# lidq92/LBDRN-MSIC

Hardware: AMD Instinct MI355X
Metric: Mpixels/s encode+decode (and bpp/PSNR parity) on D2/K5/bc64/nl2 (higher is better)
Workload: dtype f32; 1 GPU; synthetic 8-band 2048x2048 uint16 tile per step, K=5 D=2 bc=64 nl=2 bs=8192 e=10 (BASELINE.json configs[1] by default); encode fit + 16-bit weight truncation + decode; tiles_per_gpu=50, tiles_in_flight_per_gpu=4, tiles_per_launch=2, parallelism=image-sharded x1

## Files before the change

include/lbdrn_hip.h:

```cpp
#ifndef LBDRN_HIP_H
#define LBDRN_HIP_H

#include <stddef.h>
#include <stdint.h>

#ifdef __cplusplus
extern "C" {
#endif
#if defined(__GNUC__)
#pragma GCC visibility push(default)
#endif

#define LBDRN_ABI_VERSION 2

typedef enum lbdrn_status {
    LBDRN_OK = 0,
    LBDRN_E_ARG = -1,
    LBDRN_E_DEVICE = -2,
    LBDRN_E_UNSUPPORTED = -3,
    LBDRN_E_WORKSPACE = -4
} lbdrn_status;

typedef struct lbdrn_geom {
    int32_t C, H, W;
// ... 58 lines not shown

size_t lbdrn_train_workspace(const lbdrn_geom *g, const lbdrn_net *net, int32_t batch_size);
#define LBDRN_TRAIN_ALONE 0x800
int lbdrn_train_prepare(const lbdrn_geom *g, const lbdrn_net *net, const uint16_t *img,
                        const uint16_t *msb, int32_t batch_size, void *workspace,
                        size_t workspace_bytes, int32_t path, void *stream);
int lbdrn_train_epoch(const lbdrn_geom *g, const lbdrn_net *net, const uint16_t *img,
                      const uint16_t *msb, const int64_t *perm, int64_t n, int32_t batch_size,
                      float *params, float *exp_avg, float *exp_avg_sq, int64_t adam_step0,
                      double lr, float *losses, void *workspace, size_t workspace_bytes,
                      int32_t path, void *stream);

int lbdrn_train_group_max(void);
int32_t lbdrn_train_group_size(const lbdrn_geom *g, const lbdrn_net *net);
int32_t lbdrn_train_step_features(const lbdrn_geom *g, const lbdrn_net *net);
int lbdrn_train_epoch_group(int32_t count, const lbdrn_geom *const *g, const lbdrn_net *net,
                            const uint16_t *const *img, const uint16_t *const *msb, const int64_t *const *perm,
                            int64_t n, int32_t batch_size, float *const *params, float *const *exp_avg,
                            float *const *exp_avg_sq, int64_t adam_step0, double lr, float *const *losses,
                            void *const *workspace, size_t workspace_bytes, int32_t path, void *stream);

int lbdrn_train_profile_mode(int32_t mode);

size_t lbdrn_randperm_workspace(int64_t n, int32_t count);
int lbdrn_randperm(const uint64_t *seeds, int32_t count, int64_t n, int64_t *perm, void *workspace,
                   size_t workspace_bytes, void *stream);
int64_t lbdrn_mt19937_jump_poly(int32_t segment, uint32_t *poly624);

size_t lbdrn_plane_bound(int32_t C, int32_t H, int32_t W);
size_t lbdrn_plane_workspace(int32_t C, int32_t H, int32_t W);
// ... 30 lines not shown
```

lbdrn-msic_amd/csrc/cabi.hip:

```cpp
#include <string>

#include "common.hpp"

namespace lbdrn {
const char* last_error();
bool mfma_train_supported(const lbdrn_geom& g, const lbdrn_net& net, int bs = 0);
int mfma_train_step_features(const lbdrn_geom& g, const lbdrn_net& net);
bool mfma_train_takes_groups(const lbdrn_geom& g, const lbdrn_net& net);
size_t mfma_train_workspace(const lbdrn_geom& g, const lbdrn_net& net, int bs);
int mfma_train_prepare(const lbdrn_geom& g, const lbdrn_net& net, const uint16_t* img,
                       const uint16_t* msb, int bs, void* ws, size_t ws_bytes, hipStream_t s);
int mfma_train_epoch(const lbdrn_geom& g, const lbdrn_net& net, const uint16_t* img,
                     const uint16_t* msb, const int64_t* perm, int64_t n, int bs, float* params,
                     float* m, float* v, int64_t step0, double lr, float* losses, void* ws,
                     size_t ws_bytes, hipStream_t s, bool alone);
int train_profile_mode(int mode);
size_t randperm_workspace(int64_t n, int count);
size_t plane_bound(int C, int H, int W);
size_t plane_workspace(int C, int H, int W);
int plane_encode(const uint16_t* planes, int C, int H, int W, void* body, size_t body_cap, uint64_t* body_bytes,
                 void* ws, size_t ws_bytes, hipStream_t s);
int plane_decode(const void* body, size_t body_bytes, int C, int H, int W, uint16_t* planes, int* status, void* ws,
                 size_t ws_bytes, hipStream_t s);
int64_t mt19937_jump_poly(int segment, uint32_t* out);
int randperm_batch(const uint64_t* seeds, int count, int64_t n, int64_t* out, void* ws, size_t ws_bytes,
                   hipStream_t s);
int64_t jp2k_block_count(int C, int H, int W);
size_t jp2k_bound(int C, int H, int W);
size_t jp2k_workspace(int C, int H, int W);
int jp2k_encode(const uint16_t* planes, int C, int H, int W, int bits, uint8_t* out, size_t cap, size_t* nbytes, void* ws,
                size_t ws_bytes, hipStream_t s);
// ... 256 lines not shown

int lbdrn_train_group_max(void) { return 4; }

int32_t lbdrn_train_group_size(const lbdrn_geom* g, const lbdrn_net* net)
{
    if (!g || !net) return 1;
    return mfma_train_takes_groups(*g, *net) ? lbdrn_train_group_max() : 1;
}

int32_t lbdrn_train_step_features(const lbdrn_geom* g, const lbdrn_net* net)
{
    if (!g || !net) return 0;
    return mfma_train_step_features(*g, *net);
}

int lbdrn_train_epoch_group(int32_t count, const lbdrn_geom* const* g, const lbdrn_net* net, const uint16_t* const* img,
                            const uint16_t* const* msb, const int64_t* const* perm, int64_t n, int32_t batch_size,
                            float* const* params, float* const* exp_avg, float* const* exp_avg_sq, int64_t adam_step0,
                            double lr, float* const* losses, void* const* workspace, size_t workspace_bytes, int32_t path,
                            void* stream)
{
    LBDRN_REQUIRE(count >= 1 && count <= lbdrn_train_group_max(), "group of %d fits (1..%d)", count, lbdrn_train_group_max());
    LBDRN_REQUIRE(g && img && msb && perm && params && exp_avg && exp_avg_sq && workspace, "null pointer array");
    if (int rc = check_net(net)) return rc;
    for (int f = 0; f < count; ++f) {
        LBDRN_REQUIRE(g[f] && img[f] && msb[f] && perm[f] && params[f] && exp_avg[f] && exp_avg_sq[f], "null pointer (fit %d)", f);
        if (int rc = check_geom(g[f])) return rc;
        if (int rc = net_matches(g[f], net)) return rc;
        LBDRN_REQUIRE(g[f]->C == g[0]->C && g[f]->H == g[0]->H && g[f]->W == g[0]->W && g[f]->K == g[0]->K &&
                      g[f]->D == g[0]->D && g[f]->P == g[0]->P && g[f]->use_colors == g[0]->use_colors &&
// ... 116 lines not shown
```

lbdrn-msic_amd/csrc/train_mfma.hip:

```cpp
#include <atomic>
#include <cmath>
#include <cstdlib>
#include <utility>
#include <vector>

#include "common.hpp"
#include "lbdrn_math.hpp"

namespace lbdrn {

typedef float f32x4 __attribute__((ext_vector_type(4)));

constexpr int MAX_GROUP = 4;
constexpr int TB = 32;
constexpr int TBC = 64;
constexpr int HP = 68;
constexpr int TP = 36;
constexpr int OP = 20;
constexpr int RED_SLICES = 8;
constexpr int RED_LANES = 32;
constexpr int SLAB_ROT = 4;
constexpr int TRAIN_THREADS = 512;

constexpr int WB = 64;
constexpr int WAVE_THREADS = 256;
constexpr int WOP = 16;
__host__ __device__ constexpr int wave_xp(int LQ) { return LQ == 16 ? 80 : LQ == 32 ? 144 : LQ == 48 || LQ == 52 ? 208 : 272; }
constexpr int TBC_W = 64;
constexpr int WPT = 68;

struct FeatMap {
    int Fe;
    int zP, zs2, zc;
};
__host__ __device__ __forceinline__ int feat_of_slot(int j, const FeatMap& m)
{
// ... 118 lines not shown
bool mfma_train_supported(const lbdrn_geom& g, const lbdrn_net& net, int bs)
{
    TrainPlan p;
    if (make_train_plan(g, net, &p)) return bs <= 0 || slabs_addressable(p, bs);
    return wide_supported(g, net);
}

bool mfma_train_takes_groups(const lbdrn_geom& g, const lbdrn_net& net)
{
    TrainPlan p;
    return make_train_plan(g, net, &p) && p.wave == 2;
}


struct TrainWsLayout {
    size_t off_rows, off_pack, off_slab, slab_bytes, off_loss, off_stage, stage_bytes, off_map, total;
};

static TrainWsLayout train_ws_layout(const lbdrn_geom& g, const lbdrn_net& net, const TrainPlan& p, int bs)
{
    TrainWsLayout L;
    size_t o = 0;
    L.off_rows = o; o += align_up((size_t)g.H * g.W * p.RP * sizeof(float), 256);
    L.off_pack = o; o += align_up((size_t)p.pack_floats * sizeof(float), 256);
    const size_t nwg = std::max((size_t)(bs + TB - 1) / TB, 2 * ((size_t)(bs + WB - 1) / WB));
    L.slab_bytes = align_up(nwg * (size_t)p.slab_floats * sizeof(float), 256);
    L.off_slab = o; o += SLAB_ROT * L.slab_bytes;
    L.off_loss = o; o += align_up(nwg * sizeof(double), 256);
    L.stage_bytes = align_up(align_up((size_t)bs, WB) * p.RP * sizeof(float), 256);
    L.off_stage = o; o += 2 * L.stage_bytes;
    L.off_map = o; o += align_up((size_t)p.slab_floats * 4 * sizeof(int), 256);
    L.total = o;
    return L;
}

static bool slabs_addressable(const TrainPlan& p, int bs)
{
    const size_t nwg = std::max((size_t)(bs + TB - 1) / TB, 2 * ((size_t)(bs + WB - 1) / WB));
    return nwg * (size_t)p.slab_floats * sizeof(float) < ((size_t)1 << 31);
}

size_t mfma_train_workspace(const lbdrn_geom& g, const lbdrn_net& net, int bs)
// ... 222 lines not shown

constexpr int RED_AUX = 0x00;
#ifdef LBDRN_TIMELINE
constexpr int TL_SLOTS = 2048;
__device__ __forceinline__ void timeline_store(unsigned long long* tl, int slot, bool drain)
{
    if (!tl || slot >= TL_SLOTS) return;
    unsigned long long t;
    if (drain) asm volatile("s_waitcnt vmcnt(0)" ::: "memory");
    asm volatile("s_memrealtime %0\n\ts_waitcnt lgkmcnt(0)" : "=s"(t)::"memory");
    tl[slot] = t;
}
#endif
struct ReduceFit {
    const float* slabs;
    float *params, *m, *v, *packed;
    const double* loss_part;
    float* loss_out;
};
struct ReduceArgs {
    ReduceFit fit[MAX_GROUP];
    unsigned long long* tl;
    int nloss;
};

__global__ void __launch_bounds__(RED_SLICES * RED_LANES)
    k_reduce_adam(ReduceArgs R, int nwg, int slab_floats, const int4* __restrict__ map, float step_size, float bc2_sqrt,
                  double loss_count, int pairs)
{
    __shared__ __attribute__((aligned(16))) float part[RED_SLICES][4 * RED_LANES];
    __builtin_amdgcn_s_setprio(3);
#ifdef LBDRN_TIMELINE
    if (threadIdx.x == 0 && blockIdx.x == 0 && blockIdx.y == 0) timeline_store(R.tl, 1, false);
#endif
    const ReduceFit& F = R.fit[blockIdx.y];
    const float* __restrict__ slabs = F.slabs;
    float* __restrict__ params = F.params;
    float* __restrict__ m = F.m;
    float* __restrict__ v = F.v;
    float* __restrict__ packed = F.packed;
    const int l16 = threadIdx.x % RED_LANES, slice = threadIdx.x / RED_LANES;
    const int base = blockIdx.x * (4 * RED_LANES);
    int4 me = make_int4(-1, -1, -1, 0);
    float pm = 0.f, pv = 0.f, pp = 0.f;
    if (threadIdx.x < 4 * RED_LANES) {
        me = map[base + threadIdx.x];
        const int j = me.x < 0 ? 0 : me.x;
        pm = m[j]; pv = v[j]; pp = params[j];
    }
    const int per = (nwg + RED_SLICES - 1) / RED_SLICES;
    const int w0 = slice * per, w1 = min(nwg, w0 + per);
    float4 acc = make_float4(0.f, 0.f, 0.f, 0.f);
    const __amdgpu_buffer_rsrc_t srs = __builtin_amdgcn_make_buffer_rsrc(const_cast<float*>(slabs), (short)0,
                                                                         (int)((size_t)nwg * (pairs ? 2 : 1) * slab_floats * 4), 0x00020000);
    const int voff = (base + 4 * l16) * 4;
    auto slab4 = [&](int slab) -> float4 {
        typedef int v4i __attribute__((ext_vector_type(4)));
        const v4i x = __builtin_amdgcn_raw_buffer_load_b128(srs, voff + slab * slab_floats * 4, 0, RED_AUX);
        return make_float4(__int_as_float(x[0]), __int_as_float(x[1]), __int_as_float(x[2]), __int_as_float(x[3]));
    };
    int w = w0;
    if (pairs) {
        for (; w + 8 <= w1; w += 8) {
            float4 t[8], o[8];
#pragma unroll
            for (int u = 0; u < 8; ++u) {
                t[u] = slab4(2 * (w + u));
                o[u] = slab4(2 * (w + u) + 1);
            }
#pragma unroll
            for (int u = 0; u < 8; ++u) { acc.x += t[u].x + o[u].x; acc.y += t[u].y + o[u].y; acc.z += t[u].z + o[u].z; acc.w += t[u].w + o[u].w; }
        }
        for (; w < w1; ++w) {
            const float4 t = slab4(2 * w), o = slab4(2 * w + 1);
            acc.x += t.x + o.x; acc.y += t.y + o.y; acc.z += t.z + o.z; acc.w += t.w + o.w;
        }
    }
    for (; w + 16 <= w1; w += 16) {
        float4 t[16];
#pragma unroll
        for (int u = 0; u < 16; ++u) t[u] = slab4(w + u);
#pragma unroll
        for (int u = 0; u < 16; ++u) { acc.x += t[u].x; acc.y += t[u].y; acc.z += t[u].z; acc.w += t[u].w; }
    }
    for (; w < w1; ++w) {
        const float4 t = slab4(w);
        acc.x += t.x; acc.y += t.y; acc.z += t.z; acc.w += t.w;
    }
    *reinterpret_cast<float4*>(&part[slice][4 * l16]) = acc;
    __syncthreads();
    if (threadIdx.x < 4 * RED_LANES && me.x >= 0) {
        float g = part[0][threadIdx.x];
#pragma unroll
        for (int s = 1; s < RED_SLICES; ++s) g += part[s][threadIdx.x];
        const float w1c = (float)(1.0 - 0.9), b2 = 0.999f, w2c = (float)(1.0 - 0.999), eps = 1e-8f;
        float mi = pm + w1c * (g - pm);
        float vi = pv * b2 + w2c * (g * g);
        float denom = __builtin_sqrtf(vi) / bc2_sqrt + eps;
        float pi = pp + (-step_size) * (mi / denom);
        m[me.x] = mi;
        v[me.x] = vi;
        params[me.x] = pi;
        if (me.y >= 0) packed[me.y] = pi;
        if (me.z >= 0) packed[me.z] = pi;
    }
    if (blockIdx.x == 0 && threadIdx.x == 0 && F.loss_out) {
        double s = 0.0;
        if (pairs) for (int k = 0; k + 1 < R.nloss; k += 2) s += F.loss_part[k] + F.loss_part[k + 1];
        else for (int k = 0; k < R.nloss; ++k) s += F.loss_part[k];
        *F.loss_out = (float)(s / loss_count);
    }
#ifdef LBDRN_TIMELINE
    __syncthreads();
    if (threadIdx.x == 0 && blockIdx.y == 0) timeline_store(R.tl, 514 + blockIdx.x, true);
#endif
}

static void launch_reduce(const ReduceArgs& R, int blocks, int count, bool pairs, int nwg, int slab_floats, const int4* map,
                          float step_size, float bc2_sqrt, double loss_count, hipStream_t s)
{
    k_reduce_adam<<<dim3((unsigned)blocks, (unsigned)count), RED_SLICES * RED_LANES, 0, s>>>(R, nwg, slab_floats, map, step_size, bc2_sqrt,
                                                                                            loss_count, pairs ? 1 : 0);
}


struct TrainFit {
    const float* rows;
    const int64_t* perm;
    const float* params;
    const float* packed;
    float* slabs;
    double* loss_part;
};
struct TrainArgs {
    lbdrn_net net;
    TrainPlan p;
    int64_t npix;
// ... 27 lines not shown
typedef int v4i32 __attribute__((ext_vector_type(4)));
struct WtBuf {
    __amdgpu_buffer_rsrc_t r;
    float* base;
    __device__ __forceinline__ WtBuf(float* p, size_t bytes) : base(p)
    {
        r = __builtin_amdgcn_make_buffer_rsrc(p, (short)0, (int)bytes, 0x00020000);
    }
    __device__ __forceinline__ void store_plain(int float_off, float a, float b, float c, float d) const
    {
        *reinterpret_cast<float4*>(base + float_off) = make_float4(a, b, c, d);
    }
    __device__ __forceinline__ void store(int float_off, float a, float b, float c, float d) const
    {
        v4i32 v = {__float_as_int(a), __float_as_int(b), __float_as_int(c), __float_as_int(d)};
        __builtin_amdgcn_raw_buffer_store_b128(v, r, float_off * 4, 0, 16 );
    }
};

template <int N>
__device__ __forceinline__ void lds_load(const float* src, float (&dst)[N])
{
#pragma unroll
    for (int g = 0; g < N / 4; ++g) {
        float4 v = *reinterpret_cast<const float4*>(src + 4 * g);
        dst[4 * g] = v.x; dst[4 * g + 1] = v.y; dst[4 * g + 2] = v.z; dst[4 * g + 3] = v.w;
    }
}

template <int LQ, int NL>
__global__ void __launch_bounds__(TRAIN_THREADS, 2) k_train_mfma(TrainArgs A)
// ... 555 lines not shown
        return LBDRN_E_WORKSPACE;
    }
    A.net = net; A.npix = (int64_t)g.H * g.W;
    ReduceArgs R;
    for (int f = 0; f < MAX_GROUP; ++f) {
        const int k = f < count ? f : 0;
        if (!ws[k]) { set_error("null train workspace"); return LBDRN_E_WORKSPACE; }
        float* packed = (float*)((char*)ws[k] + L.off_pack);
        A.fit[f].rows = (float*)((char*)ws[k] + L.off_rows);
        A.fit[f].params = params[k];
        A.fit[f].packed = packed;
        A.fit[f].slabs = (float*)((char*)ws[k] + L.off_slab);
        A.fit[f].loss_part = (double*)((char*)ws[k] + L.off_loss);
        A.fit[f].perm = perm[k];
        R.fit[f].slabs = A.fit[f].slabs; R.fit[f].params = params[k]; R.fit[f].m = m[k]; R.fit[f].v = v[k];
        R.fit[f].packed = packed; R.fit[f].loss_part = A.fit[f].loss_part; R.fit[f].loss_out = nullptr;
        if (f < count) {
            LBDRN_HIP_TRY(hipMemsetAsync(packed, 0, (size_t)A.p.pack_floats * sizeof(float), s));
            k_pack_train<<<(unsigned)((A.p.NP + 255) / 256), 256, 0, s>>>(params[k], A.p, net.F, net.nl, net.C, packed);
            LBDRN_LAUNCH_CHECK();
        }
    }
    int4* map = (int4*)((char*)ws[0] + L.off_map);
    k_build_map<<<(unsigned)((A.p.slab_floats + 255) / 256), 256, 0, s>>>(A.p, net.F, net.nl, net.C, map);
    LBDRN_LAUNCH_CHECK();
    float* stage[2] = {(float*)((char*)ws[0] + L.off_stage), (float*)((char*)ws[0] + L.off_stage + L.stage_bytes)};
    A.stamps = nullptr;
#ifdef LBDRN_TRAIN_STAMPS
    const int max_wg = (bs + TB - 1) / TB;
    LBDRN_HIP_TRY(hipMalloc(&A.stamps, (size_t)max_wg * 8 * 16 * sizeof(unsigned long long)));
#endif
    A.tl = nullptr; R.tl = nullptr;
#ifdef LBDRN_TIMELINE
    const int tl_steps = (int)((n + bs - 1) / bs);
    unsigned long long* tl_buf = nullptr;
    {
        LBDRN_HIP_TRY(hipMalloc(&tl_buf, (size_t)tl_steps * TL_SLOTS * sizeof(unsigned long long)));
        LBDRN_HIP_TRY(hipMemset(tl_buf, 0, (size_t)tl_steps * TL_SLOTS * sizeof(unsigned long long)));
    }
#endif
    const int rows_per_wg = A.p.wave ? WB : TB;
    const bool split = (alone && count == 1 && split_available(A.p, net)) || split_only(A.p);
    const int red_blocks = A.p.slab_floats / (4 * RED_LANES);
    int64_t step = step0;
    int si = 0;
    for (int64_t first = 0; first < n; first += bs, ++si) {
        const int B = (int)std::min<int64_t>(bs, n - first);
        const int nwg = (B + rows_per_wg - 1) / rows_per_wg;
        for (int f = 0; f < MAX_GROUP; ++f) {
            const int k = f < count ? f : 0;
            A.fit[f].perm = perm[k] + first;
            R.fit[f].loss_out = (f < count && losses && losses[k]) ? losses[k] + si : nullptr;
        }
        A.batch_n = B;
        for (int f = 0; f < MAX_GROUP; ++f) {
            const int k = f < count ? f : 0;
            A.fit[f].slabs = (float*)((char*)ws[k] + L.off_slab + (size_t)(si % SLAB_ROT) * L.slab_bytes);
            R.fit[f].slabs = A.fit[f].slabs;
        }
#ifdef LBDRN_TIMELINE
        A.tl = tl_buf + (size_t)TL_SLOTS * si; R.tl = A.tl;
#endif
        A.inv = 1.0f / ((float)B * (float)net.C);
        const int64_t nextB = std::max<int64_t>(0, std::min<int64_t>(bs, n - first - bs));
        A.stage_in = si > 0 ? stage[si & 1] : nullptr;
        A.stage_out = nextB > 0 ? stage[(si + 1) & 1] : nullptr;
        if (A.p.wave) A.stage_in = nullptr, A.stage_out = nullptr;
        A.perm_next = perm[0] + first + bs;
        A.next_n = (int)nextB;
        A.touch_row_bytes = (alone && count == 1) ? TOUCH_ROW_BYTES : 0;
        const bool split_now = split && (B >= 2 || split_only(A.p));
        auto train_launch = [&]() { return split_now ? dispatch_split(A, 2 * nwg, count, s) : dispatch_train(A, nwg, count, s); };
        if (int rc = train_launch()) return rc;
        if (g_prof_mode == 2)
            if (int rc = train_launch()) return rc;
        ++step;
        const double bc1 = 1.0 - std::pow(0.9, (double)step), bc2 = 1.0 - std::pow(0.999, (double)step);
        R.nloss = split_now ? 2 * nwg : nwg;
        if (g_prof_mode != 3 && g_prof_mode != 4)
                launch_reduce(R, red_blocks, count, split_now, nwg, A.p.slab_floats, map, (float)(lr / bc1), (float)std::sqrt(bc2), (double)B * net.C, s);
        if (g_prof_mode == 1) {
            ReduceArgs R0 = R;
            for (int f = 0; f < MAX_GROUP; ++f) R0.fit[f].loss_out = nullptr;
            launch_reduce(R0, red_blocks, count, split_now, nwg, A.p.slab_floats, map, 0.0f, (float)std::sqrt(bc2), (double)B * net.C, s);
        }
        LBDRN_LAUNCH_CHECK();
    }
#ifdef LBDRN_TIMELINE
    {
        LBDRN_HIP_TRY(hipStreamSynchronize(s));
        std::vector<unsigned long long> h((size_t)tl_steps * TL_SLOTS);
        LBDRN_HIP_TRY(hipMemcpy(h.data(), tl_buf, h.size() * sizeof(unsigned long long), hipMemcpyDeviceToHost));
        (void)hipFree(tl_buf);
        double tr = 0, g1 = 0, rd = 0, g2 = 0; int cnt = 0;
        auto last = [&](int k, int lo, int hi) { unsigned long long m = 0; for (int j = lo; j < hi; ++j) m = std::max(m, h[(size_t)k * TL_SLOTS + j]); return m; };
        for (int k = 8; k + 1 < tl_steps; ++k) {
            const unsigned long long ts = h[(size_t)k * TL_SLOTS], rs = h[(size_t)k * TL_SLOTS + 1], te = last(k, 2, 514), re = last(k, 514, TL_SLOTS);
            const unsigned long long ts2 = h[(size_t)(k + 1) * TL_SLOTS];
            tr += (double)(te - ts); g1 += (double)((long long)(rs - te)); rd += (double)(re - rs); g2 += (double)((long long)(ts2 - re));
// ... 75 lines not shown
```

lbdrn-msic_amd/csrc/train_split.inc:

```
constexpr int SPB = 32;
constexpr int SP_HP = 68;
constexpr int SP_OP = 20;
constexpr int SP_PT = 36;
constexpr int SP_SM = 40;

constexpr int SP_RING = 12;
__host__ __device__ constexpr bool split_ring(int LQ) { return LQ > 64; }
__host__ __device__ constexpr int split_w0_groups(int LQ) { return split_ring(LQ) ? SP_RING : LQ / 4; }
__host__ __device__ constexpr int split_small_through(int k, int SPI) { return k * SPI < SP_SM / 4 ? k * SPI : SP_SM / 4; }

struct SplitLds { int w0, sm, x, xt, h0, red, idx, bias, h1, e, zo, zt, total; };
__host__ __device__ constexpr SplitLds split_lds(int LQ)
{
    SplitLds L{};
    const int G0 = LQ / 4, RG = split_w0_groups(LQ);
    int o = 0;
    const int over = 2 * SPB * SP_HP + SPB * SP_OP + 2 * 64 * SP_PT;
    L.w0 = o; o += RG * 4 * 256 > over ? RG * 4 * 256 : over;
    L.sm = o; o += SP_SM * 256;
    L.xt = (G0 + 1) * SGP + 16;
    L.x = o; o += 2 * L.xt;
    L.h0 = o; o += SPB * SP_HP;
    L.red = o; o += 4 + 4 * 16 + 12;
    L.idx = o; o += 4 * 256;
// ... 43 lines not shown
    const int tid = threadIdx.x, lane = tid & 63;
    const int wv = __builtin_amdgcn_readfirstlane(tid >> 6);
    const int st = wv >> 1, uh = wv & 1;
    const int i = lane & 15, q = lane >> 4;
    const int C = A.net.C;
    const float* W0s = lds + L.w0;
    const float* SMs = lds + L.sm;
    const float* Xs = lds + L.x;
    float* H0 = lds + L.h0;
    float* H1 = lds + L.h1;
    float* E = lds + L.e;
    float* Zo = lds + L.zo;
    float* ZT = lds + L.zt;
    float* red = lds + L.red;
    const unsigned lds0 = (unsigned)(size_t)(__attribute__((address_space(3))) void*)lds;
    const int wg = blockIdx.x, grp = wg >> 1, par = wg & 1;
    const int qb = (i >> 2) & 1, jr = (i & 3) + 4 * (i >> 3);
    const int rho = 16 * (2 * st + qb) + 2 * jr + par;
    const int grow = grp * WB + rho;
    const bool live = grow < A.batch_n;
    const int srow = 16 * st + i;
    const int sig = 8 * (2 * st + qb) + jr;
    const int t0 = 2 * uh;
    float* slab = F.slabs + (size_t)wg * p.slab_floats;
    const WtBuf slabw(slab, (size_t)p.slab_floats * 4);
#ifdef LBDRN_TRAIN_STAMPS
    unsigned long long stamp[16] = {};
    asm volatile("s_memrealtime %0\n\ts_waitcnt lgkmcnt(0)" : "=s"(stamp[14])::"memory");
#endif
#ifdef LBDRN_TIMELINE
    if (lane == 0 && wv == 0 && wg == 0 && blockIdx.y == 0) timeline_store(A.tl, 0, false);
// ... 363 lines not shown
            slab[p.sl_bias + TBC_W + 16 * w + lane] = s1;
        }
    }
    if (w == 3 && lane < 16)
        slab[p.sl_bias + NL * TBC_W + lane] = (red[4 + lane] + red[20 + lane]) + (red[36 + lane] + red[52 + lane]);
    asm volatile("" ::"v"(touched));
    STAMP(11); STAMP(12);
#ifdef LBDRN_TIMELINE
    if (lane == 0 && uh == 0 && blockIdx.y == 0) timeline_store(A.tl, 2 + 2 * wg + st, true);
#endif
#ifdef LBDRN_TRAIN_STAMPS
    asm volatile("s_waitcnt vmcnt(0)" ::: "memory");
    STAMP(13);
    asm volatile("s_memrealtime %0\n\ts_waitcnt lgkmcnt(0)" : "=s"(stamp[15])::"memory");
    if (lane == 0 && A.stamps)
        for (int k = 0; k < 16; ++k) A.stamps[(((size_t)blockIdx.y * gridDim.x + wg) * 4 + wv) * 16 + k] = stamp[k];
#endif
}
```

lbdrn-msic_amd/csrc/train_stream.inc:

```
constexpr int SGP = 260;
__host__ __device__ constexpr int stream_groups(int LQ) { return LQ / 4 + 1; }
__host__ __device__ constexpr int stream_rp(int LQ) { return 16 * stream_groups(LQ); }
__host__ __device__ constexpr int stream_wpx(int LQ)
{
    const int n = stream_groups(LQ) * SGP;
    return n + ((16 - n % 32) + 32) % 32;
}
constexpr int SHP = 68, SOP = 20;
constexpr int SHSZ = WB * SHP + 48;
constexpr int SZOSZ = WB * SOP + 48;
constexpr int SZTSZ = TBC_W * WPT;

constexpr int SRED = 8 + 2 * 64;
struct StreamLds { int x, stage, h0, red, h1, zo, zt, wh, wht, idx, total, small; };
__host__ __device__ constexpr StreamLds stream_lds(int LQ, int NL)
{
    StreamLds L{};
    const int G0 = LQ / 4, NST = (G0 + 2) / 2;
    L.x = 0;
    L.stage = 4 * stream_wpx(LQ);
    const int stage_end = L.stage + 4 * G0 * 256;
    const bool alias = 2 * (NST - 1) - 1 >= (SHSZ + SRED + 1023) / 1024 - 1;
    int r = alias ? L.stage + ((SHSZ + SRED + 3) & ~3) : L.stage;
    L.h1 = r; r += (NL - 1) * SHSZ;
// ... 149 lines not shown
    constexpr bool SMALL = L.small != 0;
    constexpr int NH = (NL - 1) * 16;
    static_assert(L.total * 4 <= 160 * 1024, "LDS map does not fit");
    const int tid = threadIdx.x, lane = tid & 63;
    const int w = __builtin_amdgcn_readfirstlane(tid >> 6);
    const int i = lane & 15, q = lane >> 4;
    const int C = A.net.C;
    float* Xs = lds + L.x;
    const float* ST = lds + L.stage;
    float* H0 = lds + L.h0;
    float* red = lds + L.red;
    float* ZT = lds + L.zt;
    float* Zo = lds + L.zo;
    auto Hl = [&](int l) -> float* { return l == 0 ? H0 : lds + L.h1 + (size_t)(l - 1) * SHSZ; };
    const unsigned lds0 = (unsigned)(size_t)(__attribute__((address_space(3))) void*)lds;
    const int wg = blockIdx.x, first = wg * WB;
    const int nvalid = min(WB, A.batch_n - first);
    const int srow = 16 * w + i;
    float* slab = F.slabs + (size_t)wg * p.slab_floats;
    const WtBuf slabw(slab, (size_t)p.slab_floats * 4);
    if (w == 4) {
        const float* fsrc = F.packed + p.pk_w0 + lane * 4;
        auto issue_frags = [&](int s) {
#pragma unroll
            for (int g = 2 * s; g < 2 * s + 2; ++g)
                if (g < G0)
#pragma unroll
                    for (int t = 0; t < 4; ++t) stream_dma(fsrc + 256 * (t * G0 + g), lds0 + 4u * (unsigned)(L.stage + (g * 4 + t) * 256));
        };
        if (A.batch_n >= 2) {
            const int64_t* isrc = F.perm + min(first + 2 * (lane & 31), A.batch_n - 2);
// ... 576 lines not shown
            if (half == 0) slab[p.sl_bias + u] = mine + other;
        }
        if (w == 3 && lane < 16)
            slab[p.sl_bias + NL * TBC_W + lane] = ((red[8 + lane] + red[24 + lane]) + (red[40 + lane] + red[56 + lane])) +
                                                  ((red[72 + lane] + red[88 + lane]) + (red[104 + lane] + red[120 + lane]));
    }
    STAMP(12);
#ifdef LBDRN_TIMELINE
    if (lane == 0 && blockIdx.y == 0) timeline_store(A.tl, 2 + wg * 4 + w, true);
#endif
#ifdef LBDRN_TRAIN_STAMPS
    asm volatile("s_waitcnt vmcnt(0)" ::: "memory");
    STAMP(13);
    asm volatile("s_memrealtime %0\n\ts_waitcnt lgkmcnt(0)" : "=s"(stamp[15])::"memory");
    if (lane == 0 && A.stamps)
        for (int k = 0; k < 16; ++k) A.stamps[(((size_t)blockIdx.y * gridDim.x + wg) * 4 + w) * 16 + k] = stamp[k];
#endif
}
```

lbdrn-msic_amd/csrc/train_wide.inc:

```

struct WidePlan {
    FeatMap fm;
    int LQ, NT0, RP, NT, bc, nl;
    int64_t NP;
    int64_t offW[3], offB[3];
    int pk_w0, pk_wh, pk_wl, pk_wht, pk_wlt, pack_floats;
    int sl_hid, sl_out, sl_bias, slab_floats;
    int w_dp, w_df;
    int lds_floats;
    int xo;
};

constexpr int DW_KS = 1024;
constexpr int HB = 32;

static bool make_wide_plan(const lbdrn_geom& g, const lbdrn_net& net, WidePlan* out)
{
    if (net.act != LBDRN_ACT_SINE || (net.bc != 128 && net.bc != 256) || net.nl < 1 || net.nl > 2 || net.C > 16 || net.F < 1) return false;
    WidePlan p;
    p.bc = net.bc; p.NT = net.bc / 16; p.nl = net.nl;
    p.fm = centre_skipping_map(g, net);
    p.RP = (p.fm.Fe + net.C + 3) / 4 * 4;
    p.LQ = 0;
    for (int lq : {16, 32, 48, 52, 64})
// ... 27 lines not shown
    p.w_dp = 64 / rp4;
    p.w_df = 64 % rp4;
    p.xo = (16 * p.NT0 + 63) / 64 * 64;
    {
        const int ep = net.bc + 4, r0 = std::max(HB * wave_xp(p.LQ), HB * ep);
        p.lds_floats = r0 + (net.nl > 1 ? HB * ep : 0) + 2 * HB * 20 + 4;
    }
    if ((size_t)p.lds_floats * 4 > 160 * 1024) return false;
    if (p.xo > 256) return false;
    *out = p;
    return true;
}

static int wide_plan_features(const WidePlan& p) { return p.fm.Fe; }

struct WideWsLayout { size_t off_rows, off_pack, off_slab, off_loss, off_map, off_x, off_h[2], off_dz[2], off_dzo, total; };

static WideWsLayout wide_ws_layout(const lbdrn_geom& g, const lbdrn_net& net, const WidePlan& p, int bs)
{
    WideWsLayout L;
    size_t o = 0;
    const size_t rpw = HB;
    const size_t nwg = ((size_t)bs + rpw - 1) / rpw;
    L.off_rows = o; o += align_up((size_t)g.H * g.W * p.RP * sizeof(float), 256);
    L.off_pack = o; o += align_up((size_t)p.pack_floats * sizeof(float), 256);
    const size_t nrows = (nwg * rpw + 63) / 64 * 64, nslabs = (nrows + DW_KS - 1) / DW_KS;
    L.off_slab = o; o += align_up(nslabs * (size_t)p.slab_floats * sizeof(float), 256);
    L.off_loss = o; o += align_up(nwg * sizeof(double), 256);
    L.off_map = o; o += align_up((size_t)p.slab_floats * 4 * sizeof(int), 256);
    L.off_x = o; o += align_up(nrows * (size_t)p.xo * sizeof(float), 256);
    L.off_h[1] = L.off_dz[1] = o;
    for (int l = 0; l < net.nl; ++l) {
        L.off_h[l] = o; o += align_up(nrows * (size_t)p.bc * sizeof(float), 256);
        L.off_dz[l] = o; o += align_up(nrows * (size_t)p.bc * sizeof(float), 256);
    }
    L.off_dzo = o; o += align_up(nrows * (size_t)WOP * sizeof(float), 256);
    L.total = o;
    return L;
}

__device__ __forceinline__ int2 wide_frag_pos(int64_t idx, const WidePlan& p, int F, int C)
{
// ... 727 lines not shown
        A.batch_n = B;
        A.inv = 1.0f / ((float)B * (float)net.C);
        if (int rc = dispatch_wide(A, nwg, s, false)) return rc;
        if (g_prof_mode == 2)
            if (int rc = dispatch_wide(A, nwg, s, false)) return rc;
        Dw.nrows = (nwg * rpw + 63) / 64 * 64;
        const int nslabs = Dw.nslices = (Dw.nrows + DW_KS - 1) / DW_KS;
        if (g_prof_mode != 4)
            if (int rc = dispatch_dw(Dw, s)) return rc;
        if (g_prof_mode == 5)
            if (int rc = dispatch_dw(Dw, s)) return rc;
        ++step;
        const double bc1 = 1.0 - std::pow(0.9, (double)step), bc2 = 1.0 - std::pow(0.999, (double)step);
        ReduceArgs R;
        for (int f = 0; f < MAX_GROUP; ++f)
            R.fit[f] = ReduceFit{A.slabs, params, m, v, packed, A.loss_part, losses ? losses + si : nullptr};
        R.nloss = nwg;
        R.tl = nullptr;
        if (g_prof_mode != 3 && g_prof_mode != 4)
            launch_reduce(R, A.p.slab_floats / (4 * RED_LANES), 1, false, nslabs, A.p.slab_floats, map, (float)(lr / bc1), (float)std::sqrt(bc2), (double)B * net.C, s);
        if (g_prof_mode == 1) {
            for (int f = 0; f < MAX_GROUP; ++f) R.fit[f].loss_out = nullptr;
            launch_reduce(R, A.p.slab_floats / (4 * RED_LANES), 1, false, nslabs, A.p.slab_floats, map, 0.0f, (float)std::sqrt(bc2), (double)B * net.C, s);
        }
        LBDRN_LAUNCH_CHECK();
    }
#ifdef LBDRN_TRAIN_STAMPS
    {
        LBDRN_HIP_TRY(hipStreamSynchronize(s));
        const int nw = ((int)std::min<int64_t>(bs, n) + HB - 1) / HB * 4;
        std::vector<unsigned long long> h((size_t)nw * 16);
        LBDRN_HIP_TRY(hipMemcpy(h.data(), A.stamps, h.size() * sizeof(unsigned long long), hipMemcpyDeviceToHost));
        (void)hipFree(A.stamps);
        double d[14] = {}, clk = 0;
        for (int k = 0; k < nw; ++k) {
            for (int j = 1; j <= 13; ++j) d[j] += (double)(h[k * 16 + j] - h[k * 16 + j - 1]);
            clk += (double)(h[k * 16 + 13] - h[k * 16 + 0]) / (double)(h[k * 16 + 15] - h[k * 16 + 14]) * 100.0;
        }
// ... 11 lines not shown
```

lbdrn-msic_amd/lbdrn_hip/_lib.py:

```python
import ctypes
import os

_HERE = os.path.dirname(os.path.abspath(__file__))
_LIB_PATH = os.environ.get("LBDRN_HIP_LIB") or os.path.join(os.path.dirname(_HERE), "liblbdrn_hip.so")

ABI_VERSION = 2
PATH_AUTO, PATH_GENERIC, PATH_MFMA = 0, 1, 2
EVAL_BACKGROUND = 0x200
EVAL_FAST = 0x400
EVAL_X16 = 0x1000
TRAIN_ALONE = 0x800


class LbdrnError(RuntimeError):
    code = None


E_ARG, E_DEVICE, E_UNSUPPORTED, E_WORKSPACE = -1, -2, -3, -4


class Geom(ctypes.Structure):
    _fields_ = [("C", ctypes.c_int32), ("H", ctypes.c_int32), ("W", ctypes.c_int32),
                ("K", ctypes.c_int32), ("D", ctypes.c_int32), ("msb_max", ctypes.c_int32),
                ("use_colors", ctypes.c_int32), ("relative", ctypes.c_int32),
# ... 22 lines not shown
    "lbdrn_forward": (ctypes.c_int, [_NP, _vp, _vp, _i64, _vp, _vp, _sz, _vp]),
    "lbdrn_tape_bytes": (_sz, [_NP, _i64]),
    "lbdrn_forward_tape": (ctypes.c_int, [_NP, _vp, _vp, _i64, _vp, _vp, _sz, _vp]),
    "lbdrn_backward_workspace": (_sz, [_NP, _i64]),
    "lbdrn_backward": (ctypes.c_int, [_NP, _vp, _vp, _i64, _vp, _sz, _vp, _vp, _vp, _vp, _vp, _sz, _vp]),
    "lbdrn_apply_workspace": (_sz, [_GP, _NP]),
    "lbdrn_decode_fused": (ctypes.c_int, [_GP, _NP, _vp, _vp, _vp, _vp, _vp, _sz, _i32, _vp]),
    "lbdrn_eval_sse": (ctypes.c_int, [_GP, _NP, _vp, _vp, _vp, _vp, _vp, _sz, _i32, _vp]),
    "lbdrn_train_workspace": (_sz, [_GP, _NP, _i32]),
    "lbdrn_train_prepare": (ctypes.c_int, [_GP, _NP, _vp, _vp, _i32, _vp, _sz, _i32, _vp]),
    "lbdrn_train_epoch": (ctypes.c_int, [_GP, _NP, _vp, _vp, _vp, _i64, _i32, _vp, _vp, _vp, _i64,
                                         _dbl, _vp, _vp, _sz, _i32, _vp]),
    "lbdrn_train_group_max": (ctypes.c_int, []),
    "lbdrn_train_step_features": (_i32, [_GP, _NP]),
    "lbdrn_train_group_size": (_i32, [_GP, _NP]),
    "lbdrn_train_epoch_group": (ctypes.c_int, [_i32, _vp, _NP, _vp, _vp, _vp, _i64, _i32, _vp, _vp, _vp, _i64, _dbl, _vp,
                                               _vp, _sz, _i32, _vp]),
    "lbdrn_train_profile_mode": (ctypes.c_int, [_i32]),
    "lbdrn_randperm_workspace": (_sz, [_i64, _i32]),
    "lbdrn_randperm": (ctypes.c_int, [ctypes.POINTER(ctypes.c_uint64), _i32, _i64, _vp, _vp, _sz, _vp]),
    "lbdrn_mt19937_jump_poly": (_i64, [_i32, _vp]),
    "lbdrn_plane_bound": (_sz, [_i32, _i32, _i32]),
    "lbdrn_plane_workspace": (_sz, [_i32, _i32, _i32]),
    "lbdrn_plane_encode": (ctypes.c_int, [_vp, _i32, _i32, _i32, _vp, _sz, _vp, _vp, _sz, _vp]),
    "lbdrn_plane_decode": (ctypes.c_int, [_vp, _sz, _i32, _i32, _i32, _vp, _vp, _vp, _sz, _vp]),
    "lbdrn_jp2k_block_count": (_i64, [_i32, _i32, _i32]),
    "lbdrn_jp2k_bound": (_sz, [_i32, _i32, _i32]),
    "lbdrn_jp2k_workspace": (_sz, [_i32, _i32, _i32]),
    "lbdrn_jp2k_encode": (ctypes.c_int, [_vp, _i32, _i32, _i32, _i32, _vp, _sz, ctypes.POINTER(ctypes.c_size_t), _vp, _sz, _vp]),
    "lbdrn_weights_bound": (_sz, [_i64]),
# ... 41 lines not shown
```

Before: 69.30 Mpixels/s.

## Split gradient slab reduction into parallel slice kernel plus Adam kernel, reorder workgroups

Replaces the single reduce+Adam kernel, which had each block loop over all slabs for 8 slices, with a first kernel that spreads slice partial sums across many small blocks and writes them to a new partial buffer. A second kernel sums the 8 partials and applies Adam, and when there are only a few slabs it reads them directly and skips the first kernel. Training workgroups are renumbered so consecutive block IDs map to different reduction slices, with an early exit for padding blocks. This aims to increase parallelism in the reduction, at the cost of an extra launch and extra global traffic for the partial buffer.

```diff
diff --git a/include/lbdrn_hip.h b/include/lbdrn_hip.h
--- a/include/lbdrn_hip.h
+++ b/include/lbdrn_hip.h
@@ -96,6 +96,8 @@
 int lbdrn_train_group_max(void);
 int32_t lbdrn_train_group_size(const lbdrn_geom *g, const lbdrn_net *net);
 int32_t lbdrn_train_step_features(const lbdrn_geom *g, const lbdrn_net *net);
+int32_t lbdrn_train_slice_grid(int32_t groups, int32_t split);
+int32_t lbdrn_train_slice_workgroup(int32_t groups, int32_t split, int32_t index);
 int lbdrn_train_epoch_group(int32_t count, const lbdrn_geom *const *g, const lbdrn_net *net,
                             const uint16_t *const *img, const uint16_t *const *msb, const int64_t *const *perm,
                             int64_t n, int32_t batch_size, float *const *params, float *const *exp_avg,
diff --git a/lbdrn-msic_amd/csrc/cabi.hip b/lbdrn-msic_amd/csrc/cabi.hip
--- a/lbdrn-msic_amd/csrc/cabi.hip
+++ b/lbdrn-msic_amd/csrc/cabi.hip
@@ -15,6 +15,8 @@
                      float* m, float* v, int64_t step0, double lr, float* losses, void* ws,
                      size_t ws_bytes, hipStream_t s, bool alone);
 int train_profile_mode(int mode);
+int train_slice_grid(int groups, bool split);
+int train_slice_workgroup(int groups, bool split, int b);
 size_t randperm_workspace(int64_t n, int count);
 size_t plane_bound(int C, int H, int W);
 size_t plane_workspace(int C, int H, int W);
@@ -301,6 +303,9 @@
     return mfma_train_step_features(*g, *net);
 }
 
+int32_t lbdrn_train_slice_grid(int32_t groups, int32_t split) { return train_slice_grid(groups, split != 0); }
+int32_t lbdrn_train_slice_workgroup(int32_t groups, int32_t split, int32_t index) { return train_slice_workgroup(groups, split != 0, index); }
+
 int lbdrn_train_epoch_group(int32_t count, const lbdrn_geom* const* g, const lbdrn_net* net, const uint16_t* const* img,
                             const uint16_t* const* msb, const int64_t* const* perm, int64_t n, int32_t batch_size,
                             float* const* params, float* const* exp_avg, float* const* exp_avg_sq, int64_t adam_step0,
diff --git a/lbdrn-msic_amd/csrc/train_mfma.hip b/lbdrn-msic_amd/csrc/train_mfma.hip
--- a/lbdrn-msic_amd/csrc/train_mfma.hip
+++ b/lbdrn-msic_amd/csrc/train_mfma.hip
@@ -19,7 +19,28 @@
 constexpr int OP = 20;
 constexpr int RED_SLICES = 8;
 constexpr int RED_LANES = 32;
-constexpr int SLAB_ROT = 4;
+constexpr int RED_COLS = 64;
+#ifndef AB_SLAB_ROT
+#define AB_SLAB_ROT 4
+#endif
+#ifndef AB_STORE_AUX
+#define AB_STORE_AUX 16
+#endif
+constexpr int SLAB_ROT = AB_SLAB_ROT;
+__host__ __device__ __forceinline__ int slice_per(int groups) { return (groups + RED_SLICES - 1) / RED_SLICES; }
+__host__ __device__ __forceinline__ int slice_group(int b, int per) { return (b % RED_SLICES) * per + b / RED_SLICES; }
+__host__ __device__ __forceinline__ int slice_split_wg(int b, int per)
+{
+    const int j = b / RED_SLICES;
+    return 2 * ((b % RED_SLICES) * per + (j >> 1)) + (j & 1);
+}
+int train_slice_grid(int groups, bool split) { return groups < 1 ? 0 : RED_SLICES * slice_per(groups) * (split ? 2 : 1); }
+int train_slice_workgroup(int groups, bool split, int b)
+{
+    if (groups < 1 || b < 0 || b >= train_slice_grid(groups, split)) return -1;
+    const int per = slice_per(groups), wg = split ? slice_split_wg(b, per) : slice_group(b, per);
+    return (split ? wg >> 1 : wg) < groups ? wg : -1;
+}
 constexpr int TRAIN_THREADS = 512;
 
 constexpr int WB = 64;
@@ -168,7 +189,7 @@
 
 
 struct TrainWsLayout {
-    size_t off_rows, off_pack, off_slab, slab_bytes, off_loss, off_stage, stage_bytes, off_map, total;
+    size_t off_rows, off_pack, off_slab, slab_bytes, off_part, off_loss, off_stage, stage_bytes, off_map, total;
 };
 
 static TrainWsLayout train_ws_layout(const lbdrn_geom& g, const lbdrn_net& net, const TrainPlan& p, int bs)
@@ -180,6 +201,7 @@
     const size_t nwg = std::max((size_t)(bs + TB - 1) / TB, 2 * ((size_t)(bs + WB - 1) / WB));
     L.slab_bytes = align_up(nwg * (size_t)p.slab_floats * sizeof(float), 256);
     L.off_slab = o; o += SLAB_ROT * L.slab_bytes;
+    L.off_part = o; o += align_up((size_t)RED_SLICES * p.slab_floats * sizeof(float), 256);
     L.off_loss = o; o += align_up(nwg * sizeof(double), 256);
     L.stage_bytes = align_up(align_up((size_t)bs, WB) * p.RP * sizeof(float), 256);
     L.off_stage = o; o += 2 * L.stage_bytes;
@@ -432,6 +454,7 @@
 #endif
 struct ReduceFit {
     const float* slabs;
+    float* part;
     float *params, *m, *v, *packed;
     const double* loss_part;
     float* loss_out;
@@ -442,39 +465,25 @@
     int nloss;
 };
 
-__global__ void __launch_bounds__(RED_SLICES * RED_LANES)
-    k_reduce_adam(ReduceArgs R, int nwg, int slab_floats, const int4* __restrict__ map, float step_size, float bc2_sqrt,
-                  double loss_count, int pairs)
-{
-    __shared__ __attribute__((aligned(16))) float part[RED_SLICES][4 * RED_LANES];
+__global__ void __launch_bounds__(RED_COLS)
+    k_reduce_slices(ReduceArgs R, int nwg, int slab_floats, int pairs)
+{
     __builtin_amdgcn_s_setprio(3);
 #ifdef LBDRN_TIMELINE
     if (threadIdx.x == 0 && blockIdx.x == 0 && blockIdx.y == 0) timeline_store(R.tl, 1, false);
 #endif
     const ReduceFit& F = R.fit[blockIdx.y];
-    const float* __restrict__ slabs = F.slabs;
-    float* __restrict__ params = F.params;
-    float* __restrict__ m = F.m;
-    float* __restrict__ v = F.v;
-    float* __restrict__ packed = F.packed;
-    const int l16 = threadIdx.x % RED_LANES, slice = threadIdx.x / RED_LANES;
-    const int base = blockIdx.x * (4 * RED_LANES);
-    int4 me = make_int4(-1, -1, -1, 0);
-    float pm = 0.f, pv = 0.f, pp = 0.f;
-    if (threadIdx.x < 4 * RED_LANES) {
-        me = map[base + threadIdx.x];
-        const int j = me.x < 0 ? 0 : me.x;
-        pm = m[j]; pv = v[j]; pp = params[j];
-    }
-    const int per = (nwg + RED_SLICES - 1) / RED_SLICES;
+    const int slice = blockIdx.x % RED_SLICES, lane4 = (blockIdx.x / RED_SLICES) * RED_COLS + threadIdx.x;
+    if (4 * lane4 >= slab_floats) return;
+    const int per = slice_per(nwg);
     const int w0 = slice * per, w1 = min(nwg, w0 + per);
     float4 acc = make_float4(0.f, 0.f, 0.f, 0.f);
-    const __amdgpu_buffer_rsrc_t srs = __builtin_amdgcn_make_buffer_rsrc(const_cast<float*>(slabs), (short)0,
+    const __amdgpu_buffer_rsrc_t srs = __builtin_amdgcn_make_buffer_rsrc(const_cast<float*>(F.slabs), (short)0,
                                                                          (int)((size_t)nwg * (pairs ? 2 : 1) * slab_floats * 4), 0x00020000);
-    const int voff = (base + 4 * l16) * 4;
+    const int voff = 16 * lane4;
     auto slab4 = [&](int slab) -> float4 {
         typedef int v4i __attribute__((ext_vector_type(4)));
-        const v4i x = __builtin_amdgcn_raw_buffer_load_b128(srs, voff + slab * slab_floats * 4, 0, RED_AUX);
+        const v4i x = __builtin_amdgcn_raw_buffer_load_b128(srs, voff, slab * slab_floats * 4, RED_AUX);
         return make_float4(__int_as_float(x[0]), __int_as_float(x[1]), __int_as_float(x[2]), __int_as_float(x[3]));
     };
     int w = w0;
@@ -505,12 +514,31 @@
         const float4 t = slab4(w);
         acc.x += t.x; acc.y += t.y; acc.z += t.z; acc.w += t.w;
     }
-    *reinterpret_cast<float4*>(&part[slice][4 * l16]) = acc;
-    __syncthreads();
-    if (threadIdx.x < 4 * RED_LANES && me.x >= 0) {
-        float g = part[0][threadIdx.x];
-#pragma unroll
-        for (int s = 1; s < RED_SLICES; ++s) g += part[s][threadIdx.x];
+    *reinterpret_cast<float4*>(F.part + (size_t)slice * slab_floats + 4 * lane4) = acc;
+}
+
+__global__ void __launch_bounds__(4 * RED_LANES)
+    k_reduce_adam(ReduceArgs R, int nparts, int slab_floats, const int4* __restrict__ map, float step_size, float bc2_sqrt,
+                  double loss_count, int pairs)
+{
+
+    __builtin_amdgcn_s_setprio(3);
+    const ReduceFit& F = R.fit[blockIdx.y];
+    float* __restrict__ params = F.params;
+    float* __restrict__ m = F.m;
+    float* __restrict__ v = F.v;
+    float* __restrict__ packed = F.packed;
+    const int e = blockIdx.x * (4 * RED_LANES) + threadIdx.x;
+    const int4 me = map[e];
+    if (me.x >= 0) {
+        const float pm = m[me.x], pv = v[me.x], pp = params[me.x];
+        float p8[RED_SLICES];
+#pragma unroll
+        for (int s = 0; s < RED_SLICES; ++s)
+            p8[s] = nparts == 0 ? F.part[(size_t)s * slab_floats + e] : s < nparts ? 0.0f + F.slabs[(size_t)s * slab_floats + e] : 0.0f;
+        float g = p8[0];
+#pragma unroll
+        for (int s = 1; s < RED_SLICES; ++s) g += p8[s];
         const float w1c = (float)(1.0 - 0.9), b2 = 0.999f, w2c = (float)(1.0 - 0.999), eps = 1e-8f;
         float mi = pm + w1c * (g - pm);
         float vi = pv * b2 + w2c * (g * g);
@@ -529,16 +557,18 @@
         *F.loss_out = (float)(s / loss_count);
     }
 #ifdef LBDRN_TIMELINE
-    __syncthreads();
     if (threadIdx.x == 0 && blockIdx.y == 0) timeline_store(R.tl, 514 + blockIdx.x, true);
 #endif
 }
 
-static void launch_reduce(const ReduceArgs& R, int blocks, int count, bool pairs, int nwg, int slab_floats, const int4* map,
+static void launch_reduce(const ReduceArgs& R, int count, bool pairs, int nwg, int slab_floats, const int4* map,
                           float step_size, float bc2_sqrt, double loss_count, hipStream_t s)
 {
-    k_reduce_adam<<<dim3((unsigned)blocks, (unsigned)count), RED_SLICES * RED_LANES, 0, s>>>(R, nwg, slab_floats, map, step_size, bc2_sqrt,
-                                                                                            loss_count, pairs ? 1 : 0);
+    const int cols = (slab_floats / 4 + RED_COLS - 1) / RED_COLS;
+    const bool direct = !pairs && nwg <= RED_SLICES;
+    if (!direct) k_reduce_slices<<<dim3((unsigned)(RED_SLICES * cols), (unsigned)count), RED_COLS, 0, s>>>(R, nwg, slab_floats, pairs ? 1 : 0);
+    k_reduce_adam<<<dim3((unsigned)(slab_floats / (4 * RED_LANES)), (unsigned)count), 4 * RED_LANES, 0, s>>>(R, direct ? nwg : 0, slab_floats, map, step_size,
+                                                                                                         bc2_sqrt, loss_count, pairs ? 1 : 0);
 }
 
 
@@ -596,7 +626,7 @@
     __device__ __forceinline__ void store(int float_off, float a, float b, float c, float d) const
     {
         v4i32 v = {__float_as_int(a), __float_as_int(b), __float_as_int(c), __float_as_int(d)};
-        __builtin_amdgcn_raw_buffer_store_b128(v, r, float_off * 4, 0, 16 );
+        __builtin_amdgcn_raw_buffer_store_b128(v, r, float_off * 4, 0, AB_STORE_AUX);
     }
 };
 
@@ -1182,7 +1212,7 @@
         A.fit[f].loss_part = (double*)((char*)ws[k] + L.off_loss);
         A.fit[f].perm = perm[k];
         R.fit[f].slabs = A.fit[f].slabs; R.fit[f].params = params[k]; R.fit[f].m = m[k]; R.fit[f].v = v[k];
-        R.fit[f].packed = packed; R.fit[f].loss_part = A.fit[f].loss_part; R.fit[f].loss_out = nullptr;
+        R.fit[f].packed = packed; R.fit[f].part = (float*)((char*)ws[k] + L.off_part); R.fit[f].loss_part = A.fit[f].loss_part; R.fit[f].loss_out = nullptr;
         if (f < count) {
             LBDRN_HIP_TRY(hipMemsetAsync(packed, 0, (size_t)A.p.pack_floats * sizeof(float), s));
             k_pack_train<<<(unsigned)((A.p.NP + 255) / 256), 256, 0, s>>>(params[k], A.p, net.F, net.nl, net.C, packed);
@@ -1209,7 +1239,6 @@
 #endif
     const int rows_per_wg = A.p.wave ? WB : TB;
     const bool split = (alone && count == 1 && split_available(A.p, net)) || split_only(A.p);
-    const int red_blocks = A.p.slab_floats / (4 * RED_LANES);
     int64_t step = step0;
     int si = 0;
     for (int64_t first = 0; first < n; first += bs, ++si) {
@@ -1238,7 +1267,9 @@
         A.next_n = (int)nextB;
         A.touch_row_bytes = (alone && count == 1) ? TOUCH_ROW_BYTES : 0;
         const bool split_now = split && (B >= 2 || split_only(A.p));
-        auto train_launch = [&]() { return split_now ? dispatch_split(A, 2 * nwg, count, s) : dispatch_train(A, nwg, count, s); };
+        auto train_launch = [&]() {
+            return split_now ? dispatch_split(A, train_slice_grid(nwg, true), count, s) : dispatch_train(A, A.p.wave == 2 ? train_slice_grid(nwg, false) : nwg, count, s);
+        };
         if (int rc = train_launch()) return rc;
         if (g_prof_mode == 2)
             if (int rc = train_launch()) return rc;
@@ -1246,11 +1277,11 @@
         const double bc1 = 1.0 - std::pow(0.9, (double)step), bc2 = 1.0 - std::pow(0.999, (double)step);
         R.nloss = split_now ? 2 * nwg : nwg;
         if (g_prof_mode != 3 && g_prof_mode != 4)
-                launch_reduce(R, red_blocks, count, split_now, nwg, A.p.slab_floats, map, (float)(lr / bc1), (float)std::sqrt(bc2), (double)B * net.C, s);
+                launch_reduce(R, count, split_now, nwg, A.p.slab_floats, map, (float)(lr / bc1), (float)std::sqrt(bc2), (double)B * net.C, s);
         if (g_prof_mode == 1) {
             ReduceArgs R0 = R;
             for (int f = 0; f < MAX_GROUP; ++f) R0.fit[f].loss_out = nullptr;
-            launch_reduce(R0, red_blocks, count, split_now, nwg, A.p.slab_floats, map, 0.0f, (float)std::sqrt(bc2), (double)B * net.C, s);
+            launch_reduce(R0, count, split_now, nwg, A.p.slab_floats, map, 0.0f, (float)std::sqrt(bc2), (double)B * net.C, s);
         }
         LBDRN_LAUNCH_CHECK();
     }
diff --git a/lbdrn-msic_amd/csrc/train_split.inc b/lbdrn-msic_amd/csrc/train_split.inc
--- a/lbdrn-msic_amd/csrc/train_split.inc
+++ b/lbdrn-msic_amd/csrc/train_split.inc
@@ -81,7 +81,9 @@
     float* ZT = lds + L.zt;
     float* red = lds + L.red;
     const unsigned lds0 = (unsigned)(size_t)(__attribute__((address_space(3))) void*)lds;
-    const int wg = blockIdx.x, grp = wg >> 1, par = wg & 1;
+    const int ngrp = (A.batch_n + WB - 1) / WB;
+    const int wg = slice_split_wg(blockIdx.x, slice_per(ngrp)), grp = wg >> 1, par = wg & 1;
+    if (grp >= ngrp) return;
     const int qb = (i >> 2) & 1, jr = (i & 3) + 4 * (i >> 3);
     const int rho = 16 * (2 * st + qb) + 2 * jr + par;
     const int grow = grp * WB + rho;
@@ -475,6 +477,6 @@
     STAMP(13);
     asm volatile("s_memrealtime %0\n\ts_waitcnt lgkmcnt(0)" : "=s"(stamp[15])::"memory");
     if (lane == 0 && A.stamps)
-        for (int k = 0; k < 16; ++k) A.stamps[(((size_t)blockIdx.y * gridDim.x + wg) * 4 + wv) * 16 + k] = stamp[k];
+        for (int k = 0; k < 16; ++k) A.stamps[(((size_t)blockIdx.y * 2 * ngrp + wg) * 4 + wv) * 16 + k] = stamp[k];
 #endif
 }
diff --git a/lbdrn-msic_amd/csrc/train_stream.inc b/lbdrn-msic_amd/csrc/train_stream.inc
--- a/lbdrn-msic_amd/csrc/train_stream.inc
+++ b/lbdrn-msic_amd/csrc/train_stream.inc
@@ -187,7 +187,9 @@
     float* Zo = lds + L.zo;
     auto Hl = [&](int l) -> float* { return l == 0 ? H0 : lds + L.h1 + (size_t)(l - 1) * SHSZ; };
     const unsigned lds0 = (unsigned)(size_t)(__attribute__((address_space(3))) void*)lds;
-    const int wg = blockIdx.x, first = wg * WB;
+    const int ngrp = (A.batch_n + WB - 1) / WB;
+    const int wg = slice_group(blockIdx.x, slice_per(ngrp)), first = wg * WB;
+    if (wg >= ngrp) return;
     const int nvalid = min(WB, A.batch_n - first);
     const int srow = 16 * w + i;
     float* slab = F.slabs + (size_t)wg * p.slab_floats;
@@ -794,6 +796,6 @@
     STAMP(13);
     asm volatile("s_memrealtime %0\n\ts_waitcnt lgkmcnt(0)" : "=s"(stamp[15])::"memory");
     if (lane == 0 && A.stamps)
-        for (int k = 0; k < 16; ++k) A.stamps[(((size_t)blockIdx.y * gridDim.x + wg) * 4 + w) * 16 + k] = stamp[k];
+        for (int k = 0; k < 16; ++k) A.stamps[(((size_t)blockIdx.y * ngrp + wg) * 4 + w) * 16 + k] = stamp[k];
 #endif
 }
diff --git a/lbdrn-msic_amd/csrc/train_wide.inc b/lbdrn-msic_amd/csrc/train_wide.inc
--- a/lbdrn-msic_amd/csrc/train_wide.inc
+++ b/lbdrn-msic_amd/csrc/train_wide.inc
@@ -65,7 +65,7 @@
 
 static int wide_plan_features(const WidePlan& p) { return p.fm.Fe; }
 
-struct WideWsLayout { size_t off_rows, off_pack, off_slab, off_loss, off_map, off_x, off_h[2], off_dz[2], off_dzo, total; };
+struct WideWsLayout { size_t off_rows, off_pack, off_slab, off_part, off_loss, off_map, off_x, off_h[2], off_dz[2], off_dzo, total; };
 
 static WideWsLayout wide_ws_layout(const lbdrn_geom& g, const lbdrn_net& net, const WidePlan& p, int bs)
 {
@@ -77,6 +77,7 @@
     L.off_pack = o; o += align_up((size_t)p.pack_floats * sizeof(float), 256);
     const size_t nrows = (nwg * rpw + 63) / 64 * 64, nslabs = (nrows + DW_KS - 1) / DW_KS;
     L.off_slab = o; o += align_up(nslabs * (size_t)p.slab_floats * sizeof(float), 256);
+    L.off_part = o; o += align_up((size_t)RED_SLICES * p.slab_floats * sizeof(float), 256);
     L.off_loss = o; o += align_up(nwg * sizeof(double), 256);
     L.off_map = o; o += align_up((size_t)p.slab_floats * 4 * sizeof(int), 256);
     L.off_x = o; o += align_up(nrows * (size_t)p.xo * sizeof(float), 256);
@@ -834,14 +835,14 @@
         const double bc1 = 1.0 - std::pow(0.9, (double)step), bc2 = 1.0 - std::pow(0.999, (double)step);
         ReduceArgs R;
         for (int f = 0; f < MAX_GROUP; ++f)
-            R.fit[f] = ReduceFit{A.slabs, params, m, v, packed, A.loss_part, losses ? losses + si : nullptr};
+            R.fit[f] = ReduceFit{A.slabs, (float*)((char*)ws + L.off_part), params, m, v, packed, A.loss_part, losses ? losses + si : nullptr};
         R.nloss = nwg;
         R.tl = nullptr;
         if (g_prof_mode != 3 && g_prof_mode != 4)
-            launch_reduce(R, A.p.slab_floats / (4 * RED_LANES), 1, false, nslabs, A.p.slab_floats, map, (float)(lr / bc1), (float)std::sqrt(bc2), (double)B * net.C, s);
+            launch_reduce(R, 1, false, nslabs, A.p.slab_floats, map, (float)(lr / bc1), (float)std::sqrt(bc2), (double)B * net.C, s);
         if (g_prof_mode == 1) {
             for (int f = 0; f < MAX_GROUP; ++f) R.fit[f].loss_out = nullptr;
-            launch_reduce(R, A.p.slab_floats / (4 * RED_LANES), 1, false, nslabs, A.p.slab_floats, map, 0.0f, (float)std::sqrt(bc2), (double)B * net.C, s);
+            launch_reduce(R, 1, false, nslabs, A.p.slab_floats, map, 0.0f, (float)std::sqrt(bc2), (double)B * net.C, s);
         }
         LBDRN_LAUNCH_CHECK();
     }
diff --git a/lbdrn-msic_amd/lbdrn_hip/_lib.py b/lbdrn-msic_amd/lbdrn_hip/_lib.py
--- a/lbdrn-msic_amd/lbdrn_hip/_lib.py
+++ b/lbdrn-msic_amd/lbdrn_hip/_lib.py
@@ -60,6 +60,8 @@
     "lbdrn_train_group_max": (ctypes.c_int, []),
     "lbdrn_train_step_features": (_i32, [_GP, _NP]),
     "lbdrn_train_group_size": (_i32, [_GP, _NP]),
+    "lbdrn_train_slice_grid": (_i32, [_i32, _i32]),
+    "lbdrn_train_slice_workgroup": (_i32, [_i32, _i32, _i32]),
     "lbdrn_train_epoch_group": (ctypes.c_int, [_i32, _vp, _NP, _vp, _vp, _vp, _i64, _i32, _vp, _vp, _vp, _i64, _dbl, _vp,
                                                _vp, _sz, _i32, _vp]),
     "lbdrn_train_profile_mode": (ctypes.c_int, [_i32]),
```

New measurement: 65.85 Mpixels/s. 5.0% lower.
